# Jittor/PointCloudLib

Hardware: AMD Instinct MI355X
Metric: point-clouds/sec fwd+bwd, PointNet++ SSG B=32 N=1024 (higher is better)
Workload: dtype f32; 1 GPU; PointNet++ SSG cls train step (fwd+bwd+SGD), B=32/GPU, N=1024 xyz+normal, gauss_ball clouds (BASELINE configs[1]); global_batch=32, n_points=1024, parallelism=dp1, launch=eager, grad_overlap=False, cpu_affinity=numa node 1 (gpu0), 128 cpus, world_size=1, sync_bn=False, entry_points=per-stack (pcl_mlp_stack_*_f32)

## Files before the change

### include/pcl_hip.h

```cpp
#ifndef PCL_HIP_H
#define PCL_HIP_H

#include <stddef.h>
#include <stdint.h>

#ifdef __cplusplus
extern "C" {
#endif

#define PCL_OK 0
#define PCL_EINVAL (-1)
#define PCL_EHIP (-2)
#define PCL_ENOSUP (-3)
#define PCL_EWS (-4)

int pcl_version(void);
void pcl_time_tagged_launch(void* start_event, void* stop_event, const char* tag);
void pcl_time_next_launch(void* start_event, void* stop_event);
const char* pcl_last_launch_kernel(void);
const char* pcl_last_error(void);

int pcl_optimal_block(int batch_size);

void pcl_set_fps_tuning(int threads_per_cloud, int issue_priority);
// ... 58 lines not shown
                         float* row_loc , float* row_feat ,
                         double* stats_ws, void* stream);
int pcl_group_linear_bwd_f32(const float* row_loc, const float* row_feat, int CF, const float* dU, const float* Y,
                             const float* a, const float* k1, const float* k2, const float* mu, const int32_t* row_src,
                             const int32_t* n_rows_dev , int B, int N, int C1, float* dUf,
                             float* dWx_part, float* dWf_part, float* dW0, int ldw, int off, void* stream);
int pcl_group_rows_transpose_supported(int N, int m, int ns);
int pcl_group_rows_transpose_i32(const int32_t* row_src, const int32_t* group_off, int B, int N, int m, int ns, int32_t* in_off,
                                 int32_t* in_rows, void* stream);
int pcl_group_linear_bwd_gather_supported(int C1);
void pcl_set_pointconv_paths(int bwd_w_rows);
void pcl_set_scatter_form(int gather);
int pcl_group_linear_bwd_gather_f32(const float* row_loc, const float* dU, const float* Y, const float* a, const float* k1,
                                    const float* k2, const float* mu, const int32_t* in_off, const int32_t* in_rows, int B, int N,
                                    int C1, float* dUf, float* dWx_part, float* dW0, int ldw, void* stream);

int pcl_head_layer_fwd_f32(const float* X, const float* W, const float* bias, const float* gamma, const float* beta,
                           float* running_mean, float* running_var, int R, int K, int N, int bn_mode, float eps, float momentum,
                           float slope, float* Ypre, float* OUT, float* mean_out, float* invstd_out, void* workspace,
                           size_t workspace_bytes, void* stream);
size_t pcl_head_layer_fwd_workspace_bytes(int R, int K, int N);
int pcl_head_layer_bwd_f32(const float* X, const float* W, const float* dOUT, const float* OUT, const float* Ypre,
                           const float* gamma, const float* mean, const float* invstd, int R, int K, int N, int bn_mode,
                           float slope, float* dY_ws, float* dW, float* dbias, float* dgamma, float* dbeta, float* dX,
                           void* stream);

#define PCL_HEAD_MAX_LAYERS 4
typedef struct pcl_head_layer_t {
    const float* W;
    const float* bias;
// ... 302 lines not shown
```

### pointcloudlib_amd/csrc/compact.hip

```cpp
#include "common.h"

namespace pcl {

struct GoffMulti { const int32_t* cnt[4]; int32_t* goff[4]; };
__device__ __forceinline__ void group_offsets_body(const int32_t* __restrict__ cnt, int G, int32_t* __restrict__ goff);
__global__ __launch_bounds__(1024) void group_offsets_kernel(const int32_t* __restrict__ cnt, int G, int32_t* __restrict__ goff) {
    group_offsets_body(cnt, G, goff);
}
__global__ __launch_bounds__(1024) void group_offsets_multi_kernel(const GoffMulti a, int G) {
    group_offsets_body(a.cnt[blockIdx.x], G, a.goff[blockIdx.x]);
}
__device__ __forceinline__ void group_offsets_body(const int32_t* __restrict__ cnt, int G, int32_t* __restrict__ goff) {
    __shared__ int part[1024];
    const int t = threadIdx.x;
    const int per = (G + 1023) / 1024;
    const int lo = min(t * per, G), hi = min(lo + per, G);
    int s = 0;
    for (int g = lo; g < hi; ++g) s += max(cnt[g], 1);
    part[t] = s;
    __syncthreads();
    for (int off = 1; off < 1024; off <<= 1) {
        const int v = t >= off ? part[t - off] : 0;
        __syncthreads();
        part[t] += v;
// ... 126 lines not shown
    for (int r = wv * 2; r < n; r += nw * 2) {
        const int r2 = min(r + 1, n - 1);
        const size_t d0 = (size_t)rsrc[r] * C, d1 = (size_t)rsrc[r2] * C;
        for (int c = lane; c < C; c += 64) {
            const float v0 = grows[(size_t)r * D + off + c], v1 = grows[(size_t)r2 * D + off + c];
            unsafeAtomicAdd(&gfeat[d0 + c], v0);
            if (r + 1 < n) unsafeAtomicAdd(&gfeat[d1 + c], v1);
        }
    }
}

constexpr int GL_MAXH = 4;
constexpr int GL_RPI = 4;
constexpr int GL_CF = 4;

struct DenseJob { const float* src; float* dst; int rows, cols, ldw, first, blocks; };

__global__ __launch_bounds__(256) void group_rows_meta_kernel(const float* __restrict__ xyz, const float* __restrict__ new_xyz,
                                                              const float* __restrict__ fs, int CF,
                                                              const int32_t* __restrict__ idx, const int32_t* __restrict__ cnt,
                                                              const int32_t* __restrict__ goff, int G, int N, int m, int ns,
                                                              int2* __restrict__ rmeta, int32_t* __restrict__ rsrc,
                                                              float4* __restrict__ rloc, float4* __restrict__ rfeat, DenseJob dj) {
    if ((int)blockIdx.x >= dj.first) {
        const int n = dj.rows * dj.cols;
        for (int i = ((int)blockIdx.x - dj.first) * 256 + (int)threadIdx.x; i < n; i += dj.blocks * 256) {
            const int r = i / dj.cols;
            dj.dst[i] = dj.src[(size_t)r * dj.ldw + (i - r * dj.cols)];
        }
        return;
// ... 61 lines not shown
#pragma unroll
            for (int j = 0; j < GL_RPI; ++j) {
                const int r = min(rn + j, R - 1);
                nl[j] = rloc[r]; sr[j] = Uf ? rsrc[r] : 0; nf[j] = CF ? rfeat[r] : make_float4(0.f, 0.f, 0.f, 0.f);
            }
        }
#pragma unroll
        for (int h = 0; h < NH; ++h) {
            const int ch = min(lane + 64 * h, C1 - 1);
            float u[GL_RPI];
#pragma unroll
            for (int j = 0; j < GL_RPI; ++j) u[j] = Uf ? Uf[(size_t)cs[j] * C1 + ch] : 0.f;
#pragma unroll
            for (int j = 0; j < GL_RPI; ++j) {
                if (r0 + j < R && lane + 64 * h < C1) {
                    float y = fmaf(wx[h][2], L[j].z, fmaf(wx[h][1], L[j].y, fmaf(wx[h][0], L[j].x, u[j])));
                    y = fmaf(wf[h][3], F[j].w, fmaf(wf[h][2], F[j].z, fmaf(wf[h][1], F[j].y, fmaf(wf[h][0], F[j].x, y))));
                    Y[(size_t)(r0 + j) * C1 + ch] = y;
                    const double w = (double)L[j].w;
                    ss[h] += w * (double)y; qq[h] += w * (double)y * (double)y;
                }
            }
        }
    }
#pragma unroll
    for (int h = 0; h < NH; ++h) { red[0][wave][lane + 64 * h] = ss[h]; red[1][wave][lane + 64 * h] = qq[h]; }
    __syncthreads();
    for (int ch = threadIdx.x; ch < C1; ch += 256) {
        double* dst = stats + (size_t)blockIdx.x * 2 * C1;
        dst[ch] = (red[0][0][ch] + red[0][1][ch]) + (red[0][2][ch] + red[0][3][ch]);
        dst[C1 + ch] = (red[1][0][ch] + red[1][1][ch]) + (red[1][2][ch] + red[1][3][ch]);
    }
// ... 67 lines not shown
            for (int d = 0; d < 3 + GL_CF; ++d) red[d][wave][lane + 64 * h] = gw[h][d];
        __syncthreads();
        if (dWx_part)
            for (int e = threadIdx.x; e < C1 * 3; e += 256) {
                const int ch = e / 3, d = e - ch * 3;
                dWx_part[(size_t)blockIdx.x * C1 * 3 + e] = (red[d][0][ch] + red[d][1][ch]) + (red[d][2][ch] + red[d][3][ch]);
            }
        if (dWf_part)
            for (int e = threadIdx.x; e < C1 * CF; e += 256) {
                const int ch = e / CF, d = 3 + (e - ch * CF);
                dWf_part[(size_t)blockIdx.x * C1 * CF + e] = (red[d][0][ch] + red[d][1][ch]) + (red[d][2][ch] + red[d][3][ch]);
            }
    }
}

template <int LPR>
__global__ __launch_bounds__(256) void group_linear_v4_kernel(const float* __restrict__ Uf, const float* __restrict__ Wx,
                                                              const float* __restrict__ Wfs, int CF, int ldw,
                                                              const float4* __restrict__ rloc, const float4* __restrict__ rfeat,
                                                              const int32_t* __restrict__ rsrc,
                                                              const int32_t* __restrict__ n_rows, float* __restrict__ Y,
                                                              double* __restrict__ stats) {
    constexpr int C1 = 4 * LPR, RPW = 64 / LPR, U = 4;
    __shared__ double red[2][4][C1];
    const int wave = threadIdx.x >> 6, lane = threadIdx.x & 63;
    const int cl = lane % LPR, rsub = lane / LPR, c4 = 4 * cl;
    const int R = *n_rows;
    float wx[3][4], wf[GL_CF][4];
    double ss[4], qq[4];
#pragma unroll
    for (int v = 0; v < 4; ++v) {
#pragma unroll
        for (int d = 0; d < 3; ++d) wx[d][v] = Wx ? Wx[(size_t)(c4 + v) * ldw + d] : 0.f;
#pragma unroll
        for (int f = 0; f < GL_CF; ++f) wf[f][v] = f < CF ? Wfs[(size_t)(c4 + v) * ldw + f] : 0.f;
        ss[v] = 0.0; qq[v] = 0.0;
    }
    const int stride = gridDim.x * 4 * RPW * U;
    for (int r0 = (blockIdx.x * 4 + wave) * RPW * U; r0 < R; r0 += stride) {
        float4 L[U], F[U], u[U];
#pragma unroll
        for (int j = 0; j < U; ++j) {
            const int r = min(r0 + j * RPW + rsub, R - 1);
            L[j] = rloc[r];
            F[j] = CF ? rfeat[r] : make_float4(0.f, 0.f, 0.f, 0.f);
            u[j] = Uf ? *reinterpret_cast<const float4*>(Uf + (size_t)rsrc[r] * C1 + c4) : make_float4(0.f, 0.f, 0.f, 0.f);
        }
#pragma unroll
        for (int j = 0; j < U; ++j) {
            const int r = r0 + j * RPW + rsub;
            if (r < R) {
                float y[4] = {u[j].x, u[j].y, u[j].z, u[j].w};
                const double w = (double)L[j].w;
#pragma unroll
                for (int v = 0; v < 4; ++v) {
                    float t = fmaf(wx[2][v], L[j].z, fmaf(wx[1][v], L[j].y, fmaf(wx[0][v], L[j].x, y[v])));
                    t = fmaf(wf[3][v], F[j].w, fmaf(wf[2][v], F[j].z, fmaf(wf[1][v], F[j].y, fmaf(wf[0][v], F[j].x, t))));
                    y[v] = t;
                    ss[v] += w * (double)t; qq[v] += w * (double)t * (double)t;
                }
                *reinterpret_cast<float4*>(Y + (size_t)r * C1 + c4) = make_float4(y[0], y[1], y[2], y[3]);
            }
        }
    }
#pragma unroll
    for (int v = 0; v < 4; ++v) {
#pragma unroll
        for (int off = LPR; off < 64; off <<= 1) { ss[v] += __shfl_xor(ss[v], off); qq[v] += __shfl_xor(qq[v], off); }
        if (rsub == 0) { red[0][wave][c4 + v] = ss[v]; red[1][wave][c4 + v] = qq[v]; }
    }
    __syncthreads();
    for (int ch = threadIdx.x; ch < C1; ch += 256) {
// ... 65 lines not shown
        __syncthreads();
        if (dWx_part)
            for (int e = threadIdx.x; e < C1 * 3; e += 256) {
                const int ch = e / 3, d = e - ch * 3;
                dWx_part[(size_t)blockIdx.x * C1 * 3 + e] = (red[d][0][ch] + red[d][1][ch]) + (red[d][2][ch] + red[d][3][ch]);
            }
        if (dWf_part)
            for (int e = threadIdx.x; e < C1 * CF; e += 256) {
                const int ch = e / CF, d = 3 + (e - ch * CF);
                dWf_part[(size_t)blockIdx.x * C1 * CF + e] = (red[d][0][ch] + red[d][1][ch]) + (red[d][2][ch] + red[d][3][ch]);
            }
    }
}

template <int LPR>
__global__ __launch_bounds__(256) void group_linear_bwd_gather_kernel(const float4* __restrict__ rloc, const float* __restrict__ dU,
                                                                      const float* __restrict__ Y, const float* __restrict__ a_,
                                                                      const float* __restrict__ k1_, const float* __restrict__ k2_,
                                                                      const float* __restrict__ mu_, const int32_t* __restrict__ in_off,
                                                                      const int32_t* __restrict__ in_rows, int P, float* __restrict__ dUf,
                                                                      float* __restrict__ dWx_part) {
    constexpr int C1 = 4 * LPR, PPW = 64 / LPR, U = 4;
    __shared__ float red[3][4][C1];
    const int wave = threadIdx.x >> 6, lane = threadIdx.x & 63;
    const int cl = lane % LPR, psub = lane / LPR, c4 = 4 * cl;
    const float4 a = *reinterpret_cast<const float4*>(a_ + c4), k1 = *reinterpret_cast<const float4*>(k1_ + c4);
    const float4 k2 = *reinterpret_cast<const float4*>(k2_ + c4), mu = *reinterpret_cast<const float4*>(mu_ + c4);
    float gw[3][4];
#pragma unroll
    for (int d = 0; d < 3; ++d)
// ... 13 lines not shown
#pragma unroll
            for (int j = 0; j < U; ++j) {
                L[j] = rloc[r[j]];
                du[j] = *reinterpret_cast<const float4*>(dU + (size_t)r[j] * C1 + c4);
                yv[j] = *reinterpret_cast<const float4*>(Y + (size_t)r[j] * C1 + c4);
            }
            int rn[U];
#pragma unroll
            for (int j = 0; j < U; ++j) rn[j] = in_rows[min(max(o0, min(o + PPW * U + j, o1 - 1)), last)];
#pragma unroll
            for (int j = 0; j < U; ++j) {
                if (o + j < o1) {
                    const float w = L[j].w;
                    const float d0 = fmaf(a.x, du[j].x, -w * fmaf(k2.x, yv[j].x - mu.x, k1.x)), d1 = fmaf(a.y, du[j].y, -w * fmaf(k2.y, yv[j].y - mu.y, k1.y));
                    const float d2 = fmaf(a.z, du[j].z, -w * fmaf(k2.z, yv[j].z - mu.z, k1.z)), d3 = fmaf(a.w, du[j].w, -w * fmaf(k2.w, yv[j].w - mu.w, k1.w));
                    acc.x += d0; acc.y += d1; acc.z += d2; acc.w += d3;
                    gw[0][0] = fmaf(d0, L[j].x, gw[0][0]); gw[0][1] = fmaf(d1, L[j].x, gw[0][1]); gw[0][2] = fmaf(d2, L[j].x, gw[0][2]); gw[0][3] = fmaf(d3, L[j].x, gw[0][3]);
                    gw[1][0] = fmaf(d0, L[j].y, gw[1][0]); gw[1][1] = fmaf(d1, L[j].y, gw[1][1]); gw[1][2] = fmaf(d2, L[j].y, gw[1][2]); gw[1][3] = fmaf(d3, L[j].y, gw[1][3]);
                    gw[2][0] = fmaf(d0, L[j].z, gw[2][0]); gw[2][1] = fmaf(d1, L[j].z, gw[2][1]); gw[2][2] = fmaf(d2, L[j].z, gw[2][2]); gw[2][3] = fmaf(d3, L[j].z, gw[2][3]);
                }
            }
#pragma unroll
            for (int j = 0; j < U; ++j) r[j] = rn[j];
        }
#pragma unroll
        for (int off = LPR; off < 64; off <<= 1) {
            acc.x += __shfl_xor(acc.x, off); acc.y += __shfl_xor(acc.y, off); acc.z += __shfl_xor(acc.z, off); acc.w += __shfl_xor(acc.w, off);
        }
        if (psub == 0) *reinterpret_cast<float4*>(dUf + (size_t)p * C1 + c4) = acc;
    }
// ... 270 lines not shown
    PCL_REQUIRE(B >= 1 && N >= 1 && pcl_group_linear_bwd_gather_supported(C1), "pcl_group_linear_bwd_gather_f32: bad sizes (C1 = %d: 64, 128 or 256)", C1);
    PCL_REQUIRE(al16(dU, Y, dUf), "pcl_group_linear_bwd_gather_f32: 16-byte aligned rows");
    PCL_REQUIRE(!dW0 || (dWx_part && ldw >= 3), "pcl_group_linear_bwd_gather_f32: dW0 needs dWx_part and ldw >= 3");
    hipStream_t st = as_stream(stream);
    const float4* rl = reinterpret_cast<const float4*>(row_loc);
    const dim3 grid(GL_BLOCKS), block(256);
    const int P = B * N;
    if (C1 == 64) hipLaunchKernelGGL(group_linear_bwd_gather_kernel<16>, grid, block, 0, st, rl, dU, Y, a, k1, k2, mu, in_off, in_rows, P, dUf, dWx_part);
    else if (C1 == 128) hipLaunchKernelGGL(group_linear_bwd_gather_kernel<32>, grid, block, 0, st, rl, dU, Y, a, k1, k2, mu, in_off, in_rows, P, dUf, dWx_part);
    else hipLaunchKernelGGL(group_linear_bwd_gather_kernel<64>, grid, block, 0, st, rl, dU, Y, a, k1, k2, mu, in_off, in_rows, P, dUf, dWx_part);
    int rc = check_launch("pcl_group_linear_bwd_gather_f32");
    if (rc || !dW0) return rc;
    hipLaunchKernelGGL(group_linear_dw_kernel, dim3((C1 * 3 + 3) / 4), block, 0, st, dWx_part, (const float*)nullptr, GL_BLOCKS, C1, 0, 0, ldw, dW0);
    return check_launch("pcl_group_linear_bwd_gather_f32(dW)");
}
```

### pointcloudlib_amd/csrc/stack.hip

```cpp
#include "common.h"
#include <string.h>

namespace pcl {

static inline size_t al256(size_t n) { return (n + 255) & ~(size_t)255; }

struct Carver {
    char* base; size_t off;
    explicit Carver(void* p) : base(static_cast<char*>(p)), off(0) {}
    template <typename T> T* take(size_t count) {
        T* r = base ? reinterpret_cast<T*>(base + off) : nullptr;
        off += al256(count * sizeof(T));
        return r;
    }
};

struct SaveLayout {
    float* Y[PCL_STACK_MAX_LAYERS];
    float* vec[PCL_STACK_MAX_LAYERS];
    int32_t* arg; float* ymax;
    int32_t* row_meta; int32_t* row_src; float* row_loc; float* row_feat;
    int32_t* in_off; int32_t* in_rows;
    size_t bytes;
};

static inline bool grouped_inline(const pcl_mlp_stack_t& d) { return d.grouped && d.Cf > 0 && d.Cf <= 4 && !d.need_dx; }
static inline bool grouped_wide(const pcl_mlp_stack_t& d) { return d.grouped && d.Cf > 0 && !grouped_inline(d); }
static inline int pooled_groups(const pcl_mlp_stack_t& d) { return d.grouped ? d.B * d.m : (d.pool ? d.P / d.pool : 0); }
static inline bool gather_scatter(const pcl_mlp_stack_t& d) {
    return grouped_wide(d) && pcl_group_linear_bwd_gather_supported(d.c[1]) && pcl_group_rows_transpose_supported(d.N, d.m, d.pool);
}

static SaveLayout save_layout(const pcl_mlp_stack_t& d, void* base) {
    SaveLayout s = {};
    Carver c(base);
    const int L = d.n_layers;
    for (int l = 0; l < L; ++l) {
        s.Y[l] = c.take<float>((size_t)d.P * d.c[l + 1]);
        s.vec[l] = c.take<float>((size_t)4 * d.c[l + 1]);
    }
    const int G = pooled_groups(d);
    if (G) { s.arg = c.take<int32_t>((size_t)G * d.c[L]); s.ymax = c.take<float>((size_t)G * d.c[L]); }
    if (d.grouped) {
        s.row_meta = c.take<int32_t>((size_t)d.P * 2);
        s.row_src = c.take<int32_t>((size_t)d.P);
        s.row_loc = c.take<float>((size_t)d.P * 4);
        if (grouped_inline(d)) s.row_feat = c.take<float>((size_t)d.P * 4);
        if (gather_scatter(d)) { s.in_off = c.take<int32_t>((size_t)d.B * d.N + 1); s.in_rows = c.take<int32_t>((size_t)d.P); }
    }
    s.bytes = c.off;
    return s;
}

static inline bool frag_fwd(const pcl_mlp_stack_t& d) { return !d.grouped && d.flush_k != 0; }
static inline bool use_gmax(const pcl_mlp_stack_t& d) { return !d.grouped && !d.flush_k && (d.pool == 32 || d.pool == 64); }
static inline bool fused_bwd_enabled() {
    return g_lab.fused_backward != 0;
}

struct FwdTmp {
    double* stats;
    float* Uf; double* pt_stats;
    float *gmax, *gmin; int32_t *gamax, *gamin;
// ... 1 lines not shown
};
static FwdTmp fwd_tmp(const pcl_mlp_stack_t& d, void* base) {
    FwdTmp t = {};
    Carver c(base);
    const int L = d.n_layers;
    size_t rows_max = 0;
    for (int l = 0; l < L; ++l) {
        size_t r;
        if (l == 0 && d.grouped) r = (size_t)pcl_group_linear_stat_rows(d.B, d.m) * 2 * d.c[1];
        else if (frag_fwd(d)) r = (size_t)pcl_frag_stat_rows(d.P) * 2 * d.c[l + 1];
        else r = (size_t)pcl_mlp_stat_rows(d.P, d.c[l + 1], d.grouped ? 2 : 0) * 2 * d.c[l + 1];
        if (r > rows_max) rows_max = r;
    }
    t.stats = c.take<double>(rows_max);
    if (grouped_wide(d)) {
        t.Uf = c.take<float>((size_t)d.B * d.N * d.c[1]);
        if (!d.flush_k) t.pt_stats = c.take<double>((size_t)pcl_mlp_stat_rows(d.B * d.N, d.c[1], 0) * 2 * d.c[1]);
    }
    if (use_gmax(d)) {
        const size_t n = (size_t)(d.P / d.pool) * d.c[L];
        t.gmax = c.take<float>(n); t.gmin = c.take<float>(n); t.gamax = c.take<int32_t>(n); t.gamin = c.take<int32_t>(n);
    }
    t.bytes = c.off;
    return t;
}

struct BwdTmp {
    float* gz;
    double* stats[2];
    float* dU[2];
    float* consts[2];
// ... 365 lines not shown
    const int L = d.n_layers, P = d.P;
    const int G = pooled_groups(d);
    const int32_t* rmeta = d.grouped ? s.row_meta : nullptr;
    const int32_t* nrows = d.grouped ? d.group_off + G : nullptr;
    void* st = d.stream;
    const float* cur = d.x;
    const float *in_scale = nullptr, *in_shift = nullptr;
    for (int l = 0; l < L; ++l) {
        const pcl_stack_layer_t& ly = d.layer[l];
        const int cin = d.c[l], cout = d.c[l + 1];
        float* Y = s.Y[l];
        int rows;
        if (l == 0 && d.grouped) {
            const int off = d.use_xyz ? 3 : 0, ldw = d.c[0];
            const bool inl = grouped_inline(d), wide = grouped_wide(d);
            if (wide) {
                PCL_TRY(group_linear_fwd_impl(d.xyz, d.new_xyz, nullptr, d.use_xyz ? ly.W : nullptr, nullptr, nullptr, 0, ldw, d.idx, d.cnt,
                                              d.group_off, d.B, d.N, d.m, d.pool, cout, Y, s.row_meta, s.row_src, s.row_loc, s.row_feat, t.stats,
                                              st, 1, ly.W + off, d.Wf_dense, d.Cf));
                tagf("pt%dx%d", d.Cf, cout);
                if (d.flush_k) PCL_TRY(pcl_frag_linear_fwd_f32(d.feature, d.Cf, d.Wf_dense, d.Cf, ly.bias, nullptr, nullptr, 0.f, d.B * d.N, d.Cf, cout, t.Uf, cout,
                                                               nullptr, nullptr, d.flush_k, st));
                else PCL_TRY(pcl_linear_fwd_rows_f32(d.feature, d.Wf_dense, ly.bias, nullptr, nullptr, 0.f, d.B * d.N, d.Cf, cout, t.Uf,
                                                     t.pt_stats, nullptr, nullptr, st));
            }
            if (gather_scatter(d))
                PCL_TRY(pcl_group_rows_transpose_i32(s.row_src, d.group_off, d.B, d.N, d.m, d.pool, s.in_off, s.in_rows, st));
            tagf("glin%d", cout, 0);
            PCL_TRY(group_linear_fwd_impl(d.xyz, d.new_xyz, wide ? t.Uf : nullptr, d.use_xyz ? ly.W : nullptr, inl ? d.feature : nullptr,
                                          inl ? ly.W + off : nullptr, inl ? d.Cf : 0, ldw, d.idx, d.cnt, d.group_off, d.B, d.N, d.m,
                                          d.pool, cout, Y, s.row_meta, s.row_src, s.row_loc, s.row_feat, t.stats, st, wide ? 2 : 3, nullptr,
                                          nullptr, 0));
            rows = pcl_group_linear_stat_rows(d.B, d.m);
        } else if (l == L - 1 && use_gmax(d)) {
            tagf("fwd%dx%d", cin, cout);
            PCL_TRY(pcl_linear_fwd_gmax_f32(cur, ly.W, ly.bias, in_scale, in_shift, d.slope, P, cin, cout, d.pool, Y, t.stats, t.gmax,
                                            t.gmin, t.gamax, t.gamin, st));
            rows = pcl_mlp_stat_rows(P, cout, 0);
        } else if (frag_fwd(d)) {
            tagf("fwd%dx%d", cin, cout);
            PCL_TRY(pcl_frag_linear_fwd_f32(cur, cin, ly.W, cin, ly.bias, in_scale, in_shift, d.slope, P, cin, cout, Y, cout, nullptr, t.stats, d.flush_k, st));
            rows = pcl_frag_stat_rows(P);
        } else {
            tagf("fwd%dx%d", cin, cout);
// ... 97 lines not shown
        if (fr)
            PCL_TRY(pcl_bn_bwd_dy_f32(ext_stats ? ext_stats : t.stats[cur_stats], rows, ly.gamma, mean, invstd, P, cout, ly.dgamma, ly.dbeta, a, k1, k2,
                                      ly.dbias, sparse ? nullptr : dU, s.Y[l], sparse ? s.arg : nullptr, sparse ? t.gz : nullptr, ns, P, t.dy_l[l], st));
        else if (!have_pre)
            PCL_TRY(pcl_bn_bwd_consts_f32(ext_stats ? ext_stats : t.stats[cur_stats], rows, ly.gamma, mean, invstd, P, cout, ly.dgamma, ly.dbeta, a, k1,
                                          k2, ly.dbias, st));
        if (ext_stats) { ext_stats = nullptr; cur_stats = 1 - cur_stats; }
        have_pre = false;
        if (l == 0 && d.grouped) {
            const int off = d.use_xyz ? 3 : 0, fan_in = d.c[0], C1 = cout;
            const bool inl = grouped_inline(d), wide = grouped_wide(d);
            const bool pt_pair = wide && d.need_dx && pcl_linear_bwd_pair_supported(d.B * d.N, C1, d.Cf, 0);
            const bool x_in_finish = pt_pair && gather_scatter(d) && t.dWxp;
            tagf("glinbwd%d", C1, 0);
            if (gather_scatter(d))
                PCL_TRY(pcl_group_linear_bwd_gather_f32(s.row_loc, dU, s.Y[0], a, k1, k2, mean, s.in_off, s.in_rows, d.B, d.N, C1, t.dUf, t.dWxp,
                                                        (t.dWxp && !x_in_finish) ? ly.dW : nullptr, fan_in, st));
            else
            PCL_TRY(group_linear_bwd_impl(s.row_loc, s.row_feat, inl ? d.Cf : 0, dU, s.Y[0], a, k1, k2, mean, s.row_src, nrows, d.B, d.N, C1,
                                          t.dUf, t.dWxp, t.dWfp, (t.dWxp || t.dWfp) ? ly.dW : nullptr, fan_in, off, st, true));
            if (wide) {
                float* one = t.unit;
                float* zero = one + C1;
                const int Pp = d.B * d.N;
                if (pt_pair) {
                    PCL_REQUIRE(d.dx, "pcl_mlp_stack_bwd_f32: need_dx without dx");
                    tagf("ptpair%dx%d", C1, d.Cf);
                    PCL_TRY(pcl_linear_bwd_pair_f32(t.dUf, t.dUf, one, zero, zero, zero, nullptr, nullptr, 1, d.Wf_dense, d.feature, nullptr, nullptr, 0.f, 0, Pp,
                                                    C1, d.Cf, d.dx, nullptr, 0, t.ptws, t.ptws_bytes, st));
                    PCL_TRY(pair_finish_impl(t.ptws, t.ptws_bytes, Pp, C1, d.Cf, ly.dW + off, fan_in, nullptr, 0, nullptr, nullptr, nullptr, 0,
                                             nullptr, nullptr, nullptr, nullptr, nullptr, nullptr, st,
                                             x_in_finish ? t.dWxp : nullptr, pcl_group_linear_stat_rows(d.B, d.m), C1, fan_in, ly.dW));
// ... 105 lines not shown
```

### pointcloudlib_amd/misc/mlp_hip.py

```python
import ctypes
import os

import torch

from .. import _lib, syncbn

_P = lambda t: None if t is None else t.data_ptr()
_FUSED_BWD = os.environ.get("PCL_FUSED_BWD", "1") != "0"


def _stream():
    return torch._C._cuda_getCurrentRawStream(torch.cuda.current_device())


def _rows_cost(nrows_dev, P, per_row, const):
    if nrows_dev is None:
        return per_row * P + const
    return lambda: per_row * int(nrows_dev.item()) + const


def _empty(shape, dev, dtype=torch.float32):
    return torch.empty(shape, dtype=dtype, device=dev)


# ... 416 lines not shown
        row_feat = _empty((cap, 4), dev) if inline else None
        _lib.call("pcl_group_linear_f32", _P(xyz), _P(new_xyz), _P(Uf), _P(Wx), _P(feat2) if inline else None,
                  _P(Wf) if inline else None, C if inline else 0, W0.shape[1], _P(idx), _P(cnt), _P(group_off), B, N, m, ns, C1, _P(Y),
                  _P(row_meta), _P(row_src), _P(row_loc), _P(row_feat), _P(stats), st,
                  algo_bytes=_rows_cost(group_off[B * m:], cap, 4 * C1 * (2 if Uf is not None else 1) + 36, 4 * cap), tag=f"glin{C1}")
        link.stats, link.rows = stats, rows
        in_off = in_rows = None
        if (Uf is not None and _lib.size_query("pcl_group_linear_bwd_gather_supported", C1)
                and _lib.size_query("pcl_group_rows_transpose_supported", N, m, ns)):
            in_off, in_rows = _empty((B * N + 1,), dev, torch.int32), _empty((cap,), dev, torch.int32)
            _lib.call("pcl_group_rows_transpose_i32", _P(row_src), _P(group_off), B, N, m, ns, _P(in_off), _P(in_rows), st)
        ctx.link = link
        ctx.dims = (B, N, m, ns, C1, C, off, inline, rows)
        ctx.mark_non_differentiable(row_meta, row_src)
        ctx.set_materialize_grads(False)
        ctx.save_for_backward(group_off, Y, row_src, row_loc, row_feat, feat2, None if inline else Wf, in_off, in_rows)
        return Y, row_meta, row_src

    @staticmethod
    def backward(ctx, du, *_):
        B, N, m, ns, C1, C, off, inline, rows = ctx.dims
        group_off, Y, row_src, row_loc, row_feat, feat2, Wf, in_off, in_rows = ctx.saved_tensors
        a, k1, k2, mu = ctx.link.consts
        ctx.link.consts = None
        dev = Y.device
        st = _stream()
        lib = _lib.lib()
        if du is None:
            return (None,) * 9
        need_w = ctx.needs_input_grad[3]
        wide = C > 0 and not inline
        fan_in = off + C
        dUf = _empty((B * N, C1), dev) if wide else None
        dWxp = _empty((rows, C1, 3), dev) if (off and need_w) else None
        dWfp = _empty((rows, C1, C), dev) if (inline and need_w) else None
        dW0 = _empty((C1, fan_in), dev) if need_w else None
        if dUf is not None and in_off is not None:
            _lib.call("pcl_group_linear_bwd_gather_f32", _P(row_loc), _P(du.contiguous()), _P(Y), _P(a), _P(k1), _P(k2), _P(mu), _P(in_off), _P(in_rows),
                      B, N, C1, _P(dUf), _P(dWxp), _P(dW0) if (dW0 is not None and dWxp is not None) else None, fan_in, st,
                      algo_bytes=_rows_cost(group_off[B * m:], B * m * ns, 4 * C1 * 2 + 36, 4 * B * N * C1), tag=f"glinbwd{C1}")
        elif dUf is not None or dWxp is not None or dWfp is not None:
            fin = dW0 is not None and (dWxp is not None or dWfp is not None)
            _lib.call("pcl_group_linear_bwd_f32", _P(row_loc), _P(row_feat), C if inline else 0, _P(du.contiguous()), _P(Y),
                      _P(a), _P(k1), _P(k2), _P(mu), _P(row_src), _P(group_off[B * m:]), B, N, C1, _P(dUf), _P(dWxp), _P(dWfp),
                      _P(dW0) if fin else None, fan_in, off, st,
                      algo_bytes=_rows_cost(group_off[B * m:], B * m * ns, 4 * C1 * (3 if wide else 2) + 36, 0), tag=f"glinbwd{C1}")
        dfeat = None
        if wide:
            one, zero = _const_vec(dev, C1, 1.0), _const_vec(dev, C1, 0.0)
            P = B * N
            if need_w:
                nbytes = _lib.size_query("pcl_linear_bwd_dw_workspace_bytes", P, C1, C)
                ws = _empty(((nbytes + 3) // 4,), dev)
                _lib.call("pcl_linear_bwd_dw_rows_f32", _P(dUf), _P(dUf), _P(one), _P(zero), _P(zero), _P(zero), None, None, 1,
                          _P(feat2), None, None, 0.0, P, C1, C, _P(dW0[:, off:]), _P(ws), nbytes, None, None, fan_in, st,
# ... 312 lines not shown
```

Baseline: 17860 point-clouds/s.

## Recompute grouped-linear outputs in backward instead of reading stored Y

Adds backward kernels for the grouped first layer that rebuild the pre-BN output Y for each row from the row location and features, the small weights and, on the gather path, the per-point Uf projection. This replaces reading the large per-row Y tensor during backward. The gather path now keeps Uf in the saved workspace so backward can use it. The trade is a little extra FMA work per row against removing a full read of Y (rows x C1 floats) from memory.

```diff
diff --git a/include/pcl_hip.h b/include/pcl_hip.h
--- a/include/pcl_hip.h
+++ b/include/pcl_hip.h
@@ -96,6 +96,14 @@
 int pcl_group_linear_bwd_gather_f32(const float* row_loc, const float* dU, const float* Y, const float* a, const float* k1,
                                     const float* k2, const float* mu, const int32_t* in_off, const int32_t* in_rows, int B, int N,
                                     int C1, float* dUf, float* dWx_part, float* dW0, int ldw, void* stream);
+int pcl_group_linear_bwd_regen_supported(int C1, int CF);
+int pcl_group_linear_bwd_regen_f32(const float* row_loc, const float* row_feat, const float* Wx, const float* Wf_small, int CF, int ldw,
+                                   const float* dU, const float* a, const float* k1, const float* k2, const float* mu,
+                                   const int32_t* n_rows_dev , int C1, float* dWx_part, float* dWf_part, float* dW0,
+                                   int ld0, int off, void* stream);
+int pcl_group_linear_bwd_gather_regen_f32(const float* row_loc, const float* dU, const float* Uf, const float* Wx, int ldw, const float* a,
+                                          const float* k1, const float* k2, const float* mu, const int32_t* in_off, const int32_t* in_rows,
+                                          int B, int N, int C1, float* dUf, float* dWx_part, float* dW0, int ld0, void* stream);
 
 int pcl_head_layer_fwd_f32(const float* X, const float* W, const float* bias, const float* gamma, const float* beta,
                            float* running_mean, float* running_var, int R, int K, int N, int bn_mode, float eps, float momentum,
diff --git a/pointcloudlib_amd/csrc/compact.hip b/pointcloudlib_amd/csrc/compact.hip
--- a/pointcloudlib_amd/csrc/compact.hip
+++ b/pointcloudlib_amd/csrc/compact.hip
@@ -164,6 +164,11 @@
 constexpr int GL_RPI = 4;
 constexpr int GL_CF = 4;
 
+__device__ __forceinline__ float glin_row_value(float u, const float4& L, const float4& F, const float (&wx)[3], const float (&wf)[GL_CF]) {
+    const float t = fmaf(wx[2], L.z, fmaf(wx[1], L.y, fmaf(wx[0], L.x, u)));
+    return fmaf(wf[3], F.w, fmaf(wf[2], F.z, fmaf(wf[1], F.y, fmaf(wf[0], F.x, t))));
+}
+
 struct DenseJob { const float* src; float* dst; int rows, cols, ldw, first, blocks; };
 
 __global__ __launch_bounds__(256) void group_rows_meta_kernel(const float* __restrict__ xyz, const float* __restrict__ new_xyz,
@@ -255,8 +260,7 @@
 #pragma unroll
             for (int j = 0; j < GL_RPI; ++j) {
                 if (r0 + j < R && lane + 64 * h < C1) {
-                    float y = fmaf(wx[h][2], L[j].z, fmaf(wx[h][1], L[j].y, fmaf(wx[h][0], L[j].x, u[j])));
-                    y = fmaf(wf[h][3], F[j].w, fmaf(wf[h][2], F[j].z, fmaf(wf[h][1], F[j].y, fmaf(wf[h][0], F[j].x, y))));
+                    const float y = glin_row_value(u[j], L[j], F[j], wx[h], wf[h]);
                     Y[(size_t)(r0 + j) * C1 + ch] = y;
                     const double w = (double)L[j].w;
                     ss[h] += w * (double)y; qq[h] += w * (double)y * (double)y;
@@ -354,6 +358,16 @@
     }
 }
 
+__device__ __forceinline__ void glin_load_weights(const float* __restrict__ Wx, const float* __restrict__ Wfs, int CF, int ldw, int c4,
+                                                  float (&wx)[4][3], float (&wf)[4][GL_CF]) {
+#pragma unroll
+    for (int v = 0; v < 4; ++v) {
+#pragma unroll
+        for (int d = 0; d < 3; ++d) wx[v][d] = Wx ? Wx[(size_t)(c4 + v) * ldw + d] : 0.f;
+#pragma unroll
+        for (int f = 0; f < GL_CF; ++f) wf[v][f] = f < CF ? Wfs[(size_t)(c4 + v) * ldw + f] : 0.f;
+    }
+}
 template <int LPR>
 __global__ __launch_bounds__(256) void group_linear_v4_kernel(const float* __restrict__ Uf, const float* __restrict__ Wx,
                                                               const float* __restrict__ Wfs, int CF, int ldw,
@@ -366,14 +380,14 @@
     const int wave = threadIdx.x >> 6, lane = threadIdx.x & 63;
     const int cl = lane % LPR, rsub = lane / LPR, c4 = 4 * cl;
     const int R = *n_rows;
-    float wx[3][4], wf[GL_CF][4];
+    float wx[4][3], wf[4][GL_CF];
     double ss[4], qq[4];
 #pragma unroll
     for (int v = 0; v < 4; ++v) {
 #pragma unroll
-        for (int d = 0; d < 3; ++d) wx[d][v] = Wx ? Wx[(size_t)(c4 + v) * ldw + d] : 0.f;
-#pragma unroll
-        for (int f = 0; f < GL_CF; ++f) wf[f][v] = f < CF ? Wfs[(size_t)(c4 + v) * ldw + f] : 0.f;
+        for (int d = 0; d < 3; ++d) wx[v][d] = Wx ? Wx[(size_t)(c4 + v) * ldw + d] : 0.f;
+#pragma unroll
+        for (int f = 0; f < GL_CF; ++f) wf[v][f] = f < CF ? Wfs[(size_t)(c4 + v) * ldw + f] : 0.f;
         ss[v] = 0.0; qq[v] = 0.0;
     }
     const int stride = gridDim.x * 4 * RPW * U;
@@ -394,8 +408,7 @@
                 const double w = (double)L[j].w;
 #pragma unroll
                 for (int v = 0; v < 4; ++v) {
-                    float t = fmaf(wx[2][v], L[j].z, fmaf(wx[1][v], L[j].y, fmaf(wx[0][v], L[j].x, y[v])));
-                    t = fmaf(wf[3][v], F[j].w, fmaf(wf[2][v], F[j].z, fmaf(wf[1][v], F[j].y, fmaf(wf[0][v], F[j].x, t))));
+                    const float t = glin_row_value(y[v], L[j], F[j], wx[v], wf[v]);
                     y[v] = t;
                     ss[v] += w * (double)t; qq[v] += w * (double)t * (double)t;
                 }
@@ -491,6 +504,77 @@
 }
 
 template <int LPR>
+__global__ __launch_bounds__(256) void group_linear_bwd_regen_kernel(const float4* __restrict__ rloc, const float4* __restrict__ rfeat,
+                                                                     const float* __restrict__ Wx, const float* __restrict__ Wfs, int CF,
+                                                                     int ldw, const float* __restrict__ dU, const float* __restrict__ a_,
+                                                                     const float* __restrict__ k1_, const float* __restrict__ k2_,
+                                                                     const float* __restrict__ mu_, const int32_t* __restrict__ n_rows,
+                                                                     float* __restrict__ dWx_part, float* __restrict__ dWf_part) {
+    constexpr int C1 = 4 * LPR, RPW = 64 / LPR, CH = 4, U = 3;
+    __shared__ float red[3 + GL_CF][4][C1];
+    const int wave = threadIdx.x >> 6, lane = threadIdx.x & 63;
+    const int cl = lane % LPR, rsub = lane / LPR, c4 = 4 * cl;
+    const int R = *n_rows;
+    float wx[4][3], wf[4][GL_CF];
+    float a[4], k1[4], k2[4], mu[4], gw[3 + GL_CF][4];
+    glin_load_weights(Wx, Wfs, CF, ldw, c4, wx, wf);
+#pragma unroll
+    for (int v = 0; v < 4; ++v) {
+        a[v] = a_[c4 + v]; k1[v] = k1_[c4 + v]; k2[v] = k2_[c4 + v]; mu[v] = mu_[c4 + v];
+#pragma unroll
+        for (int d = 0; d < 3 + GL_CF; ++d) gw[d][v] = 0.f;
+    }
+    const int stride = gridDim.x * 4 * RPW * CH, base = (blockIdx.x * 4 + wave) * RPW * CH;
+    for (int t0 = 0; base + (t0 / CH) * stride < R; t0 += U) {
+        float4 L[U], F[U], du[U];
+        int row[U];
+#pragma unroll
+        for (int j = 0; j < U; ++j) {
+            const int t = t0 + j;
+            row[j] = base + (t / CH) * stride + (t % CH) * RPW + rsub;
+            const int r = min(row[j], R - 1);
+            L[j] = rloc[r];
+            F[j] = CF ? rfeat[r] : make_float4(0.f, 0.f, 0.f, 0.f);
+            du[j] = *reinterpret_cast<const float4*>(dU + (size_t)r * C1 + c4);
+        }
+#pragma unroll
+        for (int j = 0; j < U; ++j) {
+            if (row[j] < R) {
+                const float dd[4] = {du[j].x, du[j].y, du[j].z, du[j].w};
+#pragma unroll
+                for (int v = 0; v < 4; ++v) {
+                    const float y = glin_row_value(0.f, L[j], F[j], wx[v], wf[v]);
+                    const float dy = fmaf(a[v], dd[v], -L[j].w * fmaf(k2[v], y - mu[v], k1[v]));
+                    gw[0][v] = fmaf(dy, L[j].x, gw[0][v]); gw[1][v] = fmaf(dy, L[j].y, gw[1][v]); gw[2][v] = fmaf(dy, L[j].z, gw[2][v]);
+                    gw[3][v] = fmaf(dy, F[j].x, gw[3][v]); gw[4][v] = fmaf(dy, F[j].y, gw[4][v]);
+                    gw[5][v] = fmaf(dy, F[j].z, gw[5][v]); gw[6][v] = fmaf(dy, F[j].w, gw[6][v]);
+                }
+            }
+        }
+    }
+#pragma unroll
+    for (int d = 0; d < 3 + GL_CF; ++d)
+#pragma unroll
+        for (int v = 0; v < 4; ++v) {
+            float t = gw[d][v];
+#pragma unroll
+            for (int off = LPR; off < 64; off <<= 1) t += __shfl_xor(t, off);
+            if (rsub == 0) red[d][wave][c4 + v] = t;
+        }
+    __syncthreads();
+    if (dWx_part)
+        for (int e = threadIdx.x; e < C1 * 3; e += 256) {
+            const int ch = e / 3, d = e - ch * 3;
+            dWx_part[(size_t)blockIdx.x * C1 * 3 + e] = (red[d][0][ch] + red[d][1][ch]) + (red[d][2][ch] + red[d][3][ch]);
+        }
+    if (dWf_part)
+        for (int e = threadIdx.x; e < C1 * CF; e += 256) {
+            const int ch = e / CF, d = 3 + (e - ch * CF);
+            dWf_part[(size_t)blockIdx.x * C1 * CF + e] = (red[d][0][ch] + red[d][1][ch]) + (red[d][2][ch] + red[d][3][ch]);
+        }
+}
+
+template <int LPR>
 __global__ __launch_bounds__(256) void group_linear_bwd_gather_kernel(const float4* __restrict__ rloc, const float* __restrict__ dU,
                                                                       const float* __restrict__ Y, const float* __restrict__ a_,
                                                                       const float* __restrict__ k1_, const float* __restrict__ k2_,
@@ -534,6 +618,88 @@
                     const float w = L[j].w;
                     const float d0 = fmaf(a.x, du[j].x, -w * fmaf(k2.x, yv[j].x - mu.x, k1.x)), d1 = fmaf(a.y, du[j].y, -w * fmaf(k2.y, yv[j].y - mu.y, k1.y));
                     const float d2 = fmaf(a.z, du[j].z, -w * fmaf(k2.z, yv[j].z - mu.z, k1.z)), d3 = fmaf(a.w, du[j].w, -w * fmaf(k2.w, yv[j].w - mu.w, k1.w));
+                    acc.x += d0; acc.y += d1; acc.z += d2; acc.w += d3;
+                    gw[0][0] = fmaf(d0, L[j].x, gw[0][0]); gw[0][1] = fmaf(d1, L[j].x, gw[0][1]); gw[0][2] = fmaf(d2, L[j].x, gw[0][2]); gw[0][3] = fmaf(d3, L[j].x, gw[0][3]);
+                    gw[1][0] = fmaf(d0, L[j].y, gw[1][0]); gw[1][1] = fmaf(d1, L[j].y, gw[1][1]); gw[1][2] = fmaf(d2, L[j].y, gw[1][2]); gw[1][3] = fmaf(d3, L[j].y, gw[1][3]);
+                    gw[2][0] = fmaf(d0, L[j].z, gw[2][0]); gw[2][1] = fmaf(d1, L[j].z, gw[2][1]); gw[2][2] = fmaf(d2, L[j].z, gw[2][2]); gw[2][3] = fmaf(d3, L[j].z, gw[2][3]);
+                }
+            }
+#pragma unroll
+            for (int j = 0; j < U; ++j) r[j] = rn[j];
+        }
+#pragma unroll
+        for (int off = LPR; off < 64; off <<= 1) {
+            acc.x += __shfl_xor(acc.x, off); acc.y += __shfl_xor(acc.y, off); acc.z += __shfl_xor(acc.z, off); acc.w += __shfl_xor(acc.w, off);
+        }
+        if (psub == 0) *reinterpret_cast<float4*>(dUf + (size_t)p * C1 + c4) = acc;
+    }
+    if (dWx_part) {
+#pragma unroll
+        for (int d = 0; d < 3; ++d)
+#pragma unroll
+            for (int v = 0; v < 4; ++v) {
+                float t = gw[d][v];
+#pragma unroll
+                for (int off = LPR; off < 64; off <<= 1) t += __shfl_xor(t, off);
+                if (psub == 0) red[d][wave][c4 + v] = t;
+            }
+        __syncthreads();
+        for (int e = threadIdx.x; e < C1 * 3; e += 256) {
+            const int ch = e / 3, d = e - ch * 3;
+            dWx_part[(size_t)blockIdx.x * C1 * 3 + e] = (red[d][0][ch] + red[d][1][ch]) + (red[d][2][ch] + red[d][3][ch]);
+        }
+    }
+}
+
+template <int LPR>
+__global__ __launch_bounds__(256) void group_linear_bwd_gather_regen_kernel(const float4* __restrict__ rloc, const float* __restrict__ dU,
+                                                                      const float* __restrict__ Uf, const float* __restrict__ Wx, int ldw,
+                                                                      const float* __restrict__ a_,
+                                                                      const float* __restrict__ k1_, const float* __restrict__ k2_,
+                                                                      const float* __restrict__ mu_, const int32_t* __restrict__ in_off,
+                                                                      const int32_t* __restrict__ in_rows, int P, float* __restrict__ dUf,
+                                                                      float* __restrict__ dWx_part) {
+    constexpr int C1 = 4 * LPR, PPW = 64 / LPR, U = 4;
+    __shared__ float red[3][4][C1];
+    const int wave = threadIdx.x >> 6, lane = threadIdx.x & 63;
+    const int cl = lane % LPR, psub = lane / LPR, c4 = 4 * cl;
+    const float4 a = *reinterpret_cast<const float4*>(a_ + c4), k1 = *reinterpret_cast<const float4*>(k1_ + c4);
+    const float4 k2 = *reinterpret_cast<const float4*>(k2_ + c4), mu = *reinterpret_cast<const float4*>(mu_ + c4);
+    float gw[3][4], wx[4][3], wf[4][GL_CF];
+    glin_load_weights(Wx, nullptr, 0, ldw, c4, wx, wf);
+    const float4 F0 = make_float4(0.f, 0.f, 0.f, 0.f);
+#pragma unroll
+    for (int d = 0; d < 3; ++d)
+#pragma unroll
+        for (int v = 0; v < 4; ++v) gw[d][v] = 0.f;
+    const int stride = gridDim.x * 4;
+    const int last = max(in_off[P] - 1, 0);
+    for (int p = blockIdx.x * 4 + wave; p < P; p += stride) {
+        const int o0 = in_off[p], o1 = in_off[p + 1];
+        float4 acc = make_float4(0.f, 0.f, 0.f, 0.f);
+        const float4 u = *reinterpret_cast<const float4*>(Uf + (size_t)p * C1 + c4);
+        int o = o0 + psub * U;
+        int r[U];
+#pragma unroll
+        for (int j = 0; j < U; ++j) r[j] = in_rows[min(max(o0, min(o + j, o1 - 1)), last)];
+        for (; o < o1; o += PPW * U) {
+            float4 L[U], du[U];
+#pragma unroll
+            for (int j = 0; j < U; ++j) {
+                L[j] = rloc[r[j]];
+                du[j] = *reinterpret_cast<const float4*>(dU + (size_t)r[j] * C1 + c4);
+            }
+            int rn[U];
+#pragma unroll
+            for (int j = 0; j < U; ++j) rn[j] = in_rows[min(max(o0, min(o + PPW * U + j, o1 - 1)), last)];
+#pragma unroll
+            for (int j = 0; j < U; ++j) {
+                if (o + j < o1) {
+                    const float w = L[j].w;
+                    const float4 yv = make_float4(glin_row_value(u.x, L[j], F0, wx[0], wf[0]), glin_row_value(u.y, L[j], F0, wx[1], wf[1]),
+                                                  glin_row_value(u.z, L[j], F0, wx[2], wf[2]), glin_row_value(u.w, L[j], F0, wx[3], wf[3]));
+                    const float d0 = fmaf(a.x, du[j].x, -w * fmaf(k2.x, yv.x - mu.x, k1.x)), d1 = fmaf(a.y, du[j].y, -w * fmaf(k2.y, yv.y - mu.y, k1.y));
+                    const float d2 = fmaf(a.z, du[j].z, -w * fmaf(k2.z, yv.z - mu.z, k1.z)), d3 = fmaf(a.w, du[j].w, -w * fmaf(k2.w, yv.w - mu.w, k1.w));
                     acc.x += d0; acc.y += d1; acc.z += d2; acc.w += d3;
                     gw[0][0] = fmaf(d0, L[j].x, gw[0][0]); gw[0][1] = fmaf(d1, L[j].x, gw[0][1]); gw[0][2] = fmaf(d2, L[j].x, gw[0][2]); gw[0][3] = fmaf(d3, L[j].x, gw[0][3]);
                     gw[1][0] = fmaf(d0, L[j].y, gw[1][0]); gw[1][1] = fmaf(d1, L[j].y, gw[1][1]); gw[1][2] = fmaf(d2, L[j].y, gw[1][2]); gw[1][3] = fmaf(d3, L[j].y, gw[1][3]);
@@ -834,3 +1000,55 @@
     hipLaunchKernelGGL(group_linear_dw_kernel, dim3((C1 * 3 + 3) / 4), block, 0, st, dWx_part, (const float*)nullptr, GL_BLOCKS, C1, 0, 0, ldw, dW0);
     return check_launch("pcl_group_linear_bwd_gather_f32(dW)");
 }
+
+extern "C" int pcl_group_linear_bwd_regen_supported(int C1, int CF) {
+    return (C1 == 64 || C1 == 128 || C1 == 256) && CF >= 0 && CF <= GL_CF;
+}
+extern "C" int pcl_group_linear_bwd_regen_f32(const float* row_loc, const float* row_feat, const float* Wx, const float* Wf_small, int CF,
+                                              int ldw, const float* dU, const float* a, const float* k1, const float* k2, const float* mu,
+                                              const int32_t* n_rows_dev, int C1, float* dWx_part, float* dWf_part, float* dW0, int ld0, int off,
+                                              void* stream) {
+    PCL_REQUIRE(row_loc && dU && a && k1 && k2 && mu && n_rows_dev, "pcl_group_linear_bwd_regen_f32: null pointer");
+    PCL_REQUIRE(pcl_group_linear_bwd_regen_supported(C1, CF), "pcl_group_linear_bwd_regen_f32: C1 = %d (64, 128 or 256), CF = %d (<= %d)", C1, CF, GL_CF);
+    PCL_REQUIRE(Wx || CF > 0, "pcl_group_linear_bwd_regen_f32: need the forward's weights (Wx and/or Wf_small)");
+    PCL_REQUIRE(CF == 0 || (row_feat && Wf_small), "pcl_group_linear_bwd_regen_f32: CF=%d inline features need row_feat and Wf_small", CF);
+    PCL_REQUIRE(ldw >= (Wx ? 3 : 0) && ldw >= CF, "pcl_group_linear_bwd_regen_f32: ldw=%d", ldw);
+    PCL_REQUIRE(dWx_part || dWf_part, "pcl_group_linear_bwd_regen_f32: nothing to compute");
+    PCL_REQUIRE(!dWf_part || CF >= 1, "pcl_group_linear_bwd_regen_f32: dWf_part needs CF >= 1");
+    PCL_REQUIRE(al16(dU, row_loc, row_feat), "pcl_group_linear_bwd_regen_f32: 16-byte aligned rows");
+    PCL_REQUIRE(!dW0 || (ld0 >= (dWx_part ? 3 : 0) && off >= 0 && ld0 >= off + (dWf_part ? CF : 0)),
+                "pcl_group_linear_bwd_regen_f32: dW0 needs ld0=%d >= off=%d + CF", ld0, off);
+    hipStream_t st = as_stream(stream);
+    const float4* rl = reinterpret_cast<const float4*>(row_loc);
+    const float4* rf = reinterpret_cast<const float4*>(row_feat);
+    const dim3 grid(GL_BLOCKS), block(256);
+    if (C1 == 64) hipLaunchKernelGGL(group_linear_bwd_regen_kernel<16>, grid, block, 0, st, rl, rf, Wx, Wf_small, CF, ldw, dU, a, k1, k2, mu, n_rows_dev, dWx_part, dWf_part);
+    else if (C1 == 128) hipLaunchKernelGGL(group_linear_bwd_regen_kernel<32>, grid, block, 0, st, rl, rf, Wx, Wf_small, CF, ldw, dU, a, k1, k2, mu, n_rows_dev, dWx_part, dWf_part);
+    else hipLaunchKernelGGL(group_linear_bwd_regen_kernel<64>, grid, block, 0, st, rl, rf, Wx, Wf_small, CF, ldw, dU, a, k1, k2, mu, n_rows_dev, dWx_part, dWf_part);
+    int rc = check_launch("pcl_group_linear_bwd_regen_f32");
+    if (rc || !dW0) return rc;
+    const int n = (dWx_part ? C1 * 3 : 0) + (dWf_part ? C1 * CF : 0);
+    hipLaunchKernelGGL(group_linear_dw_kernel, dim3((n + 3) / 4), block, 0, st, dWx_part, dWf_part, GL_BLOCKS, C1, CF, off, ld0, dW0);
+    return check_launch("pcl_group_linear_bwd_regen_f32(dW)");
+}
+extern "C" int pcl_group_linear_bwd_gather_regen_f32(const float* row_loc, const float* dU, const float* Uf, const float* Wx, int ldw,
+                                                     const float* a, const float* k1, const float* k2, const float* mu, const int32_t* in_off,
+                                                     const int32_t* in_rows, int B, int N, int C1, float* dUf, float* dWx_part, float* dW0,
+                                                     int ld0, void* stream) {
+    PCL_REQUIRE(row_loc && dU && Uf && a && k1 && k2 && mu && in_off && in_rows && dUf, "pcl_group_linear_bwd_gather_regen_f32: null pointer");
+    PCL_REQUIRE(B >= 1 && N >= 1 && pcl_group_linear_bwd_gather_supported(C1), "pcl_group_linear_bwd_gather_regen_f32: bad sizes (C1 = %d: 64, 128 or 256)", C1);
+    PCL_REQUIRE(al16(dU, Uf, dUf, row_loc) && al16(a, k1, k2, mu), "pcl_group_linear_bwd_gather_regen_f32: 16-byte aligned rows");
+    PCL_REQUIRE(!Wx || ldw >= 3, "pcl_group_linear_bwd_gather_regen_f32: ldw=%d", ldw);
+    PCL_REQUIRE(!dW0 || (dWx_part && ld0 >= 3), "pcl_group_linear_bwd_gather_regen_f32: dW0 needs dWx_part and ld0 >= 3");
+    hipStream_t st = as_stream(stream);
+    const float4* rl = reinterpret_cast<const float4*>(row_loc);
+    const dim3 grid(GL_BLOCKS), block(256);
+    const int P = B * N;
+    if (C1 == 64) hipLaunchKernelGGL(group_linear_bwd_gather_regen_kernel<16>, grid, block, 0, st, rl, dU, Uf, Wx, ldw, a, k1, k2, mu, in_off, in_rows, P, dUf, dWx_part);
+    else if (C1 == 128) hipLaunchKernelGGL(group_linear_bwd_gather_regen_kernel<32>, grid, block, 0, st, rl, dU, Uf, Wx, ldw, a, k1, k2, mu, in_off, in_rows, P, dUf, dWx_part);
+    else hipLaunchKernelGGL(group_linear_bwd_gather_regen_kernel<64>, grid, block, 0, st, rl, dU, Uf, Wx, ldw, a, k1, k2, mu, in_off, in_rows, P, dUf, dWx_part);
+    int rc = check_launch("pcl_group_linear_bwd_gather_regen_f32");
+    if (rc || !dW0) return rc;
+    hipLaunchKernelGGL(group_linear_dw_kernel, dim3((C1 * 3 + 3) / 4), block, 0, st, dWx_part, (const float*)nullptr, GL_BLOCKS, C1, 0, 0, ld0, dW0);
+    return check_launch("pcl_group_linear_bwd_gather_regen_f32(dW)");
+}
diff --git a/pointcloudlib_amd/csrc/stack.hip b/pointcloudlib_amd/csrc/stack.hip
--- a/pointcloudlib_amd/csrc/stack.hip
+++ b/pointcloudlib_amd/csrc/stack.hip
@@ -21,6 +21,7 @@
     int32_t* arg; float* ymax;
     int32_t* row_meta; int32_t* row_src; float* row_loc; float* row_feat;
     int32_t* in_off; int32_t* in_rows;
+    float* Uf;
     size_t bytes;
 };
 
@@ -46,7 +47,10 @@
         s.row_src = c.take<int32_t>((size_t)d.P);
         s.row_loc = c.take<float>((size_t)d.P * 4);
         if (grouped_inline(d)) s.row_feat = c.take<float>((size_t)d.P * 4);
-        if (gather_scatter(d)) { s.in_off = c.take<int32_t>((size_t)d.B * d.N + 1); s.in_rows = c.take<int32_t>((size_t)d.P); }
+        if (gather_scatter(d)) {
+            s.in_off = c.take<int32_t>((size_t)d.B * d.N + 1); s.in_rows = c.take<int32_t>((size_t)d.P);
+            s.Uf = c.take<float>((size_t)d.B * d.N * d.c[1]);
+        }
     }
     s.bytes = c.off;
     return s;
@@ -78,7 +82,7 @@
     }
     t.stats = c.take<double>(rows_max);
     if (grouped_wide(d)) {
-        t.Uf = c.take<float>((size_t)d.B * d.N * d.c[1]);
+        if (!gather_scatter(d)) t.Uf = c.take<float>((size_t)d.B * d.N * d.c[1]);
         if (!d.flush_k) t.pt_stats = c.take<double>((size_t)pcl_mlp_stat_rows(d.B * d.N, d.c[1], 0) * 2 * d.c[1]);
     }
     if (use_gmax(d)) {
@@ -474,20 +478,21 @@
         if (l == 0 && d.grouped) {
             const int off = d.use_xyz ? 3 : 0, ldw = d.c[0];
             const bool inl = grouped_inline(d), wide = grouped_wide(d);
+            float* const Uf = s.Uf ? s.Uf : t.Uf;
             if (wide) {
                 PCL_TRY(group_linear_fwd_impl(d.xyz, d.new_xyz, nullptr, d.use_xyz ? ly.W : nullptr, nullptr, nullptr, 0, ldw, d.idx, d.cnt,
                                               d.group_off, d.B, d.N, d.m, d.pool, cout, Y, s.row_meta, s.row_src, s.row_loc, s.row_feat, t.stats,
                                               st, 1, ly.W + off, d.Wf_dense, d.Cf));
                 tagf("pt%dx%d", d.Cf, cout);
-                if (d.flush_k) PCL_TRY(pcl_frag_linear_fwd_f32(d.feature, d.Cf, d.Wf_dense, d.Cf, ly.bias, nullptr, nullptr, 0.f, d.B * d.N, d.Cf, cout, t.Uf, cout,
+                if (d.flush_k) PCL_TRY(pcl_frag_linear_fwd_f32(d.feature, d.Cf, d.Wf_dense, d.Cf, ly.bias, nullptr, nullptr, 0.f, d.B * d.N, d.Cf, cout, Uf, cout,
                                                                nullptr, nullptr, d.flush_k, st));
-                else PCL_TRY(pcl_linear_fwd_rows_f32(d.feature, d.Wf_dense, ly.bias, nullptr, nullptr, 0.f, d.B * d.N, d.Cf, cout, t.Uf,
+                else PCL_TRY(pcl_linear_fwd_rows_f32(d.feature, d.Wf_dense, ly.bias, nullptr, nullptr, 0.f, d.B * d.N, d.Cf, cout, Uf,
                                                      t.pt_stats, nullptr, nullptr, st));
             }
             if (gather_scatter(d))
                 PCL_TRY(pcl_group_rows_transpose_i32(s.row_src, d.group_off, d.B, d.N, d.m, d.pool, s.in_off, s.in_rows, st));
             tagf("glin%d", cout, 0);
-            PCL_TRY(group_linear_fwd_impl(d.xyz, d.new_xyz, wide ? t.Uf : nullptr, d.use_xyz ? ly.W : nullptr, inl ? d.feature : nullptr,
+            PCL_TRY(group_linear_fwd_impl(d.xyz, d.new_xyz, wide ? Uf : nullptr, d.use_xyz ? ly.W : nullptr, inl ? d.feature : nullptr,
                                           inl ? ly.W + off : nullptr, inl ? d.Cf : 0, ldw, d.idx, d.cnt, d.group_off, d.B, d.N, d.m,
                                           d.pool, cout, Y, s.row_meta, s.row_src, s.row_loc, s.row_feat, t.stats, st, wide ? 2 : 3, nullptr,
                                           nullptr, 0));
@@ -615,8 +620,12 @@
             const bool x_in_finish = pt_pair && gather_scatter(d) && t.dWxp;
             tagf("glinbwd%d", C1, 0);
             if (gather_scatter(d))
-                PCL_TRY(pcl_group_linear_bwd_gather_f32(s.row_loc, dU, s.Y[0], a, k1, k2, mean, s.in_off, s.in_rows, d.B, d.N, C1, t.dUf, t.dWxp,
-                                                        (t.dWxp && !x_in_finish) ? ly.dW : nullptr, fan_in, st));
+                PCL_TRY(pcl_group_linear_bwd_gather_regen_f32(s.row_loc, dU, s.Uf, d.use_xyz ? ly.W : nullptr, fan_in, a, k1, k2, mean, s.in_off,
+                                                              s.in_rows, d.B, d.N, C1, t.dUf, t.dWxp,
+                                                              (t.dWxp && !x_in_finish) ? ly.dW : nullptr, fan_in, st));
+            else if (!t.dUf && (t.dWxp || t.dWfp) && pcl_group_linear_bwd_regen_supported(C1, inl ? d.Cf : 0) && al16(dU))
+                PCL_TRY(pcl_group_linear_bwd_regen_f32(s.row_loc, s.row_feat, d.use_xyz ? ly.W : nullptr, inl ? ly.W + off : nullptr, inl ? d.Cf : 0,
+                                                       fan_in, dU, a, k1, k2, mean, nrows, C1, t.dWxp, t.dWfp, ly.dW, fan_in, off, st));
             else
             PCL_TRY(group_linear_bwd_impl(s.row_loc, s.row_feat, inl ? d.Cf : 0, dU, s.Y[0], a, k1, k2, mean, s.row_src, nrows, d.B, d.N, C1,
                                           t.dUf, t.dWxp, t.dWfp, (t.dWxp || t.dWfp) ? ly.dW : nullptr, fan_in, off, st, true));
diff --git a/pointcloudlib_amd/misc/mlp_hip.py b/pointcloudlib_amd/misc/mlp_hip.py
--- a/pointcloudlib_amd/misc/mlp_hip.py
+++ b/pointcloudlib_amd/misc/mlp_hip.py
@@ -454,13 +454,13 @@
         ctx.dims = (B, N, m, ns, C1, C, off, inline, rows)
         ctx.mark_non_differentiable(row_meta, row_src)
         ctx.set_materialize_grads(False)
-        ctx.save_for_backward(group_off, Y, row_src, row_loc, row_feat, feat2, None if inline else Wf, in_off, in_rows)
+        ctx.save_for_backward(group_off, Y, row_src, row_loc, row_feat, feat2, None if inline else Wf, in_off, in_rows, W0, Uf)
         return Y, row_meta, row_src
 
     @staticmethod
     def backward(ctx, du, *_):
         B, N, m, ns, C1, C, off, inline, rows = ctx.dims
-        group_off, Y, row_src, row_loc, row_feat, feat2, Wf, in_off, in_rows = ctx.saved_tensors
+        group_off, Y, row_src, row_loc, row_feat, feat2, Wf, in_off, in_rows, W0, Uf = ctx.saved_tensors
         a, k1, k2, mu = ctx.link.consts
         ctx.link.consts = None
         dev = Y.device
@@ -475,10 +475,16 @@
         dWxp = _empty((rows, C1, 3), dev) if (off and need_w) else None
         dWfp = _empty((rows, C1, C), dev) if (inline and need_w) else None
         dW0 = _empty((C1, fan_in), dev) if need_w else None
+        Wx = W0[:, :3] if off else None
         if dUf is not None and in_off is not None:
-            _lib.call("pcl_group_linear_bwd_gather_f32", _P(row_loc), _P(du.contiguous()), _P(Y), _P(a), _P(k1), _P(k2), _P(mu), _P(in_off), _P(in_rows),
-                      B, N, C1, _P(dUf), _P(dWxp), _P(dW0) if (dW0 is not None and dWxp is not None) else None, fan_in, st,
-                      algo_bytes=_rows_cost(group_off[B * m:], B * m * ns, 4 * C1 * 2 + 36, 4 * B * N * C1), tag=f"glinbwd{C1}")
+            _lib.call("pcl_group_linear_bwd_gather_regen_f32", _P(row_loc), _P(du.contiguous()), _P(Uf), _P(Wx), fan_in, _P(a), _P(k1), _P(k2), _P(mu),
+                      _P(in_off), _P(in_rows), B, N, C1, _P(dUf), _P(dWxp), _P(dW0) if (dW0 is not None and dWxp is not None) else None, fan_in, st,
+                      algo_bytes=_rows_cost(group_off[B * m:], B * m * ns, 4 * C1 + 36, 8 * B * N * C1), tag=f"glinbwd{C1}")
+        elif (dUf is None and (dWxp is not None or dWfp is not None)
+              and _lib.size_query("pcl_group_linear_bwd_regen_supported", C1, C if inline else 0)):
+            _lib.call("pcl_group_linear_bwd_regen_f32", _P(row_loc), _P(row_feat), _P(Wx), _P(W0[:, off:]) if inline else None, C if inline else 0,
+                      fan_in, _P(du.contiguous()), _P(a), _P(k1), _P(k2), _P(mu), _P(group_off[B * m:]), C1, _P(dWxp), _P(dWfp), _P(dW0),
+                      fan_in, off, st, algo_bytes=_rows_cost(group_off[B * m:], B * m * ns, 4 * C1 + 36, 0), tag=f"glinbwd{C1}")
         elif dUf is not None or dWxp is not None or dWfp is not None:
             fin = dW0 is not None and (dWxp is not None or dWfp is not None)
             _lib.call("pcl_group_linear_bwd_f32", _P(row_loc), _P(row_feat), C if inline else 0, _P(du.contiguous()), _P(Y),
```

After: 18190 point-clouds/s, median of 6. 1.02x the previous value.
